# tky823/ssspy

Measured on AMD Instinct MI355X. Metric: GaussILRMA-IP1 update_once mixture-iterations/sec (F=1025,T=512,N=4,K=16), higher is better.
Workload: dtype f64; 1 GPU; BASELINE configs[1] GaussILRMA-IP1/MM (N=M=4, F=1025, T=512, n_basis=16) x 128 independent mixtures per GPU (configs[4] shard), record_loss=False, update_once() = one fused C-ABI call; batch_per_gpu=128, global_batch=128, n_bins=1025, n_frames=512, n_basis=16, parallelism=mixtures sharded, no collective, input=nmf_mixture(seed=1000+b) per mixture b (SURVEY 8d)

## Files before the change

include/ssspy_amd.h:

```cpp
#ifndef SSSPY_AMD_H
#define SSSPY_AMD_H

#include <stddef.h>

#ifdef __cplusplus
extern "C" {
#endif

enum {
  SSSPY_OK = 0,
  SSSPY_ERR_BADARG = 1,
  SSSPY_ERR_HIP = 2,
  SSSPY_ERR_UNSUPPORTED = 3,
  SSSPY_ERR_INTERNAL = 4,
};

enum { SSSPY_FLOOR_NONE = 0, SSSPY_FLOOR_MAX = 1, SSSPY_FLOOR_ADD = 2 };

enum {
  SSSPY_WEIGHT_UNIT = 0,
  SSSPY_WEIGHT_FRAME = 1,
  SSSPY_WEIGHT_BIN_FRAME = 2,
};

// ... 183 lines not shown
int ssspy_ilrma_deferred_logdet_slots(int B, int N, int F, int T, int K, double domain,
                                      int source_model);
int ssspy_ilrma_ip1_update_loss_slots(const void *X, const void *C, void *W, double *basis,
                                      double *activation, void *U, int B, int N, int F, int T,
                                      int K, double domain, int source_model, double model_param,
                                      int normalize, int floor_kind, double floor_eps,
                                      void *workspace, size_t workspace_bytes, int *info,
                                      double *slots, long long slot_stride, double *logdet,
                                      void *stream);
size_t ssspy_fold_scalar_slots_workspace_bytes(long long total, int nslots);
int ssspy_fold_scalar_slots(const double *slots, long long total, int nslots, double *out,
                            void *workspace, size_t workspace_bytes, void *stream);

enum {
  SSSPY_ROUTE_LATENCY = 0,
  SSSPY_ROUTE_THROUGHPUT = 1,
  SSSPY_ROUTE_GROUPED = 2,
  SSSPY_ROUTE_GENERIC = 3,
  SSSPY_ROUTE_WIDE_BASIS = 4,
  SSSPY_ROUTE_RUNTIME_N = 5,
};
int ssspy_ilrma_route(int B, int N, int F, int T, int K, double domain, int source_model,
                      int *act_chunks, int *basis_plan);

int ssspy_ipa_sweep(void *Vc, void *G, int B, int F, int N, int normalization, int max_iter,
                    int floor_kind, double floor_eps, int *info, void *newton_ws,
                    int *not_converged, void *stream);
size_t ssspy_ipa_sweep_newton_words(int B, int N);
int ssspy_debug_barrier_timeouts(void);

int ssspy_ilrma_partition_expand(const double *basis, const double *activation,
                                 const double *latent, double *Teff, double *Vrep, int B, int N,
                                 int F, int T, int K, void *stream);

enum { SSSPY_PARTITION_LATENT = 1, SSSPY_PARTITION_BASIS = 2, SSSPY_PARTITION_ACTIVATION = 4 };

int ssspy_ilrma_partition_update(const void *X, const void *W, double *basis, double *activation,
                                 double *latent, double *Teff, double *Vrep, int B, int N, int F,
                                 int T, int K, double domain, int source_model, double model_param,
                                 int steps, int floor_kind, double floor_eps, void *workspace,
                                 size_t workspace_bytes, void *stream);

int ssspy_ilrma_partition_normalize(void *W, const void *C, void *Y, double *basis, double *latent,
                                    int B, int N, int F, int T, int K, double domain,
                                    int floor_kind, double floor_eps, void *workspace,
                                    size_t workspace_bytes, void *stream);
// ... 450 lines not shown
```

ssspy_amd/_lib.py:

```python

import ctypes
import os

import numpy as np

_PKG = os.path.dirname(os.path.abspath(__file__))
LIB_PATH = os.environ.get("SSSPY_AMD_LIB") or os.path.join(_PKG, "lib", "libssspy_amd.so")

OK, ERR_BADARG, ERR_HIP, ERR_UNSUPPORTED, ERR_INTERNAL = 0, 1, 2, 3, 4
FLOOR_NONE, FLOOR_MAX, FLOOR_ADD = 0, 1, 2
WEIGHT_UNIT, WEIGHT_FRAME, WEIGHT_BIN_FRAME = 0, 1, 2
SOURCE_GAUSS, SOURCE_T, SOURCE_GGD = 0, 1, 2
PARTITION_LATENT, PARTITION_BASIS, PARTITION_ACTIVATION = 1, 2, 4
SOURCE_ME = 0x100
CONTRAST_LAPLACE, CONTRAST_GAUSS, CONTRAST_GAUSS_FIXED = 0, 1, 2
WHITEN, PCA_FIRST_COMPONENT_LAST, PCA_FIRST_COMPONENT_FIRST = 0, 1, 2
IPSDTA_QUAD, IPSDTA_BASIS, IPSDTA_ACT, IPSDTA_COV = range(4)
IPSDTA_MAX_SOURCES, IPSDTA_MAX_BLOCK, IPSDTA_MAX_BASIS = 8, 8, 32
(ROUTE_LATENCY, ROUTE_THROUGHPUT, ROUTE_GROUPED, ROUTE_GENERIC, ROUTE_WIDE_BASIS,
 ROUTE_RUNTIME_N) = range(6)
MNMF_ROUTE_TILED, MNMF_ROUTE_GENERIC, MNMF_ROUTE_RUNTIME = range(3)
MNMF_PLAN_FIELDS = ("fast", "ksmall", "basis_copy", "glds_cov", "glds_spatial", "kq", "handover",
                    "tail_full", "tail_tail", "tail_split", "tail_groups", "htail_full", "htail_tail",
                    "htail_split", "htail_groups", "act_chunks", "ip1_records", "spatial_fold_in_norm",
# ... 70 lines not shown
    "ssspy_ilrma_weighted_covariance": (_i, [_p, _p, _p, _p, _p, _i, _i, _i, _i, _i, _d, _i, _d, _i,
                                             _d, _p, _z, _p]),
    "ssspy_ilrma_normalize_filter": (_i, [_p, _p, _p, _i, _i, _i, _i, _d, _i, _d, _p, _z, _p]),
    "ssspy_ilrma_normalize_output": (_i, [_p, _p, _p, _i, _i, _i, _i, _i, _d, _i, _d, _p, _z, _p]),
    "ssspy_ilrma_normalize_output_tracked": (_i, [_p, _p, _p, _i, _i, _i, _i, _i, _d, _i, _d, _p, _z,
                                                  _p, _p]),
    "ssspy_ilrma_iss_weight": (_i, [_p, _p, _p, _p, _i, _i, _i, _i, _i, _d, _i, _d, _i, _d, _p]),
    "ssspy_ilrma_iss_weight_power": (_i, [_p, _p, _p, _p, _i, _i, _i, _i, _i, _d, _i, _d, _i, _d, _p]),
    "ssspy_ilrma_loss_workspace_bytes": (_z, [_i, _i, _i, _i, _i, _i]),
    "ssspy_ilrma_loss_data": (_i, [_p, _p, _p, _p, _p, _i, _i, _i, _i, _i, _d, _i, _d, _p, _z, _p]),
    "ssspy_ilrma_ip1_update": (_i, [_p, _p, _p, _p, _p, _p, _i, _i, _i, _i, _i, _d, _i, _d, _i, _i, _d,
                                    _p, _z, _p, _p]),
    "ssspy_ilrma_deferred_loss_supported": (_i, [_i, _i, _i, _i, _d, _i]),
    "ssspy_ilrma_ip1_update_deferred_loss": (_i, [_p, _p, _p, _p, _p, _p, _i, _i, _i, _i, _i, _d, _i,
                                                  _d, _i, _i, _d, _p, _z, _p, _p, _p, _p]),
    "ssspy_ilrma_deferred_loss_slots": (_i, [_i, _i, _i, _i, _i, _d, _i]),
    "ssspy_ilrma_deferred_logdet_slots": (_i, [_i, _i, _i, _i, _i, _d, _i]),
    "ssspy_ilrma_ip1_update_loss_slots": (_i, [_p, _p, _p, _p, _p, _p, _i, _i, _i, _i, _i, _d, _i,
                                               _d, _i, _i, _d, _p, _z, _p, _p, _q, _p, _p]),
    "ssspy_fold_scalar_slots_workspace_bytes": (_z, [_q, _i]),
    "ssspy_fold_scalar_slots": (_i, [_p, _q, _i, _p, _p, _z, _p]),
    "ssspy_ilrma_route": (_i, [_i, _i, _i, _i, _i, _d, _i, ctypes.POINTER(ctypes.c_int),
                                ctypes.POINTER(ctypes.c_int)]),
    "ssspy_ilrma_partition_expand": (_i, [_p, _p, _p, _p, _p, _i, _i, _i, _i, _i, _p]),
    "ssspy_ilrma_partition_update": (_i, [_p, _p, _p, _p, _p, _p, _p, _i, _i, _i, _i, _i, _d, _i, _d,
                                          _i, _i, _d, _p, _z, _p]),
    "ssspy_ilrma_partition_normalize": (_i, [_p, _p, _p, _p, _p, _i, _i, _i, _i, _i, _d, _i, _d, _p,
                                             _z, _p]),
    "ssspy_iva_frame_power_workspace_bytes": (_z, [_i, _i, _i, _i]),
    "ssspy_iva_frame_power": (_i, [_p, _p, _p, _i, _i, _i, _i, _p, _z, _p]),
    "ssspy_separate_frame_power": (_i, [_p, _p, _p, _p, _i, _i, _i, _i, _p, _z, _p]),
    "ssspy_iva_weight": (_i, [_p, _p, _p, _i, _i, _i, _i, _i, _i, _d, _p]),
    "ssspy_iva_loss_data": (_i, [_p, _p, _p, _i, _i, _i, _i, _i, _p]),
    "ssspy_iva_score_weight": (_i, [_p, _p, _p, _i, _i, _i, _i, _i, _i, _d, _p]),
    "ssspy_iva_grad_step_logdet_slots": (_i, [_i, _i, _i]),
    "ssspy_iva_grad_step": (_i, [_p, _p, _i, _i, _i, _i, _i, _i, _d, _p, _p, _q, _p]),
    "ssspy_fdica_weight": (_i, [_p, _p, _i, _i, _i, _i, _i, _i, _d, _p, _q, _p]),
    "ssspy_fdica_route": (_i, [_i, _i, _i, _i, _i]),
    "ssspy_fdica_steps": (_i, [_p, _p, _i, _i, _i, _i, _i, _i, _d, _i, _d, _i, _p, _p, _q, _p, _p]),
    "ssspy_ica_chunk_samples": (_i, [_i, _q]),
    "ssspy_ica_workspace_bytes": (_z, [_i, _i, _q]),
    "ssspy_ica_stats": (_i, [_p, _p, _p, _p, _p, _z, _i, _i, _q, _i, _i, _p]),
    "ssspy_ica_step": (_i, [_p, _z, _p, _i, _i, _q, _i, _i, _d, _p, _p, _p, _p, _p]),
    "ssspy_ica_separate": (_i, [_p, _p, _p, _i, _i, _q, _p]),
    "ssspy_prox_neg_logdet": (_i, [_p, _p, _q, _i, _d, _p]),
    "ssspy_pdsbss_contract": (_i, [_p, _p, _p, _i, _i, _i, _i, _i, _p]),
# ... 147 lines not shown
```

ssspy_amd/_ops.py:

```python

from . import _device as dv
from . import _lib, _routes
from ._device import ptr


def _L():
    return _lib.load()


import os as _os

_CANARY_DOUBLES = 4096 if _os.environ.get("SSSPY_AMD_WS_CANARY") else 0
_CANARY_VALUE = -7.25e300
_canaries = []


def _workspace(nbytes, dev):
    n = (int(nbytes) + 7) // 8
    buf = dv.empty((n + _CANARY_DOUBLES,), dv.f64, dev)
    if not _CANARY_DOUBLES:
        return buf, int(nbytes)
    import weakref

    buf[n:].fill_(_CANARY_VALUE)
# ... 491 lines not shown
        ptr(X), ptr(C), ptr(W), ptr(basis), ptr(activation), ptr(U), B, N, F, T, K, domain, model[0],
        model[1], int(bool(normalize)), flooring[0], flooring[1], ptr(ws), ws_bytes, ptr(info),
        ptr(slots), int(slot_stride), ptr(logdet), _st()), "ilrma_ip1_update_loss_slots")


def fold_scalar_slots(slots, total, nslots, out):
    ws, ws_bytes = _scratch(_L().ssspy_fold_scalar_slots_workspace_bytes(int(total), int(nslots)),
                            slots.device)
    _lib.check(_L().ssspy_fold_scalar_slots(ptr(slots), int(total), int(nslots), ptr(out), ptr(ws),
                                            ws_bytes, _st()), "fold_scalar_slots")
    return out


def ilrma_route(B, N, F, T, K, domain, model=GAUSS):
    import ctypes

    chunks = ctypes.c_int(0)
    plan = (ctypes.c_int * 3)()
    route = int(_L().ssspy_ilrma_route(B, N, F, T, K, float(domain), model[0], ctypes.byref(chunks),
                                       plan))
    if route < 0:
        raise ValueError("ilrma_route: bad shape")
    return route, int(chunks.value), tuple(plan)


def ilrma_partition_expand(basis, activation, latent, Teff, Vrep):
    B, N, F, K = Teff.shape
    T = Vrep.shape[-1]
    _lib.check(
        _L().ssspy_ilrma_partition_expand(ptr(basis), ptr(activation), ptr(latent), ptr(Teff),
                                          ptr(Vrep), B, N, F, T, K, _st()),
        "ilrma_partition_expand",
    )


def ilrma_partition_update(X, W, basis, activation, latent, Teff, Vrep, domain, steps, flooring, ws,
                           ws_bytes, model=GAUSS):
    B, N, F, T = X.shape
    K = basis.shape[-1]
    _lib.check(
        _L().ssspy_ilrma_partition_update(ptr(X), ptr(W), ptr(basis), ptr(activation), ptr(latent),
                                          ptr(Teff), ptr(Vrep), B, N, F, T, K, domain, model[0],
                                          model[1], steps, flooring[0], flooring[1], ptr(ws),
                                          ws_bytes, _st()),
        "ilrma_partition_update",
    )
# ... 922 lines not shown
```

ssspy_amd/csrc/ilrma_api.hip:

```cpp
#include "ilrma_plan.hpp"

namespace ssspy {

static inline int check_model(int source_model, double param, double domain = 2.0) {
  const int model = source_model & 0xff;
  const bool me = (source_model & SSSPY_SOURCE_ME) != 0;
  if ((source_model & ~(0xff | SSSPY_SOURCE_ME)) != 0)
    return fail(SSSPY_ERR_BADARG, "bad source model flags");
  if (me && (domain != 2.0 || model == SSSPY_SOURCE_GGD))
    return fail(SSSPY_ERR_BADARG, "ME source updates need domain == 2 and a Gauss or t model");
  if (model == SSSPY_SOURCE_GAUSS) return SSSPY_OK;
  if (model == SSSPY_SOURCE_T && param > 0.0) return SSSPY_OK;
  if (model == SSSPY_SOURCE_GGD && param > 0.0 && param < 2.0) return SSSPY_OK;
  return fail(SSSPY_ERR_BADARG, "bad source model / model_param (t: dof > 0, GGD: 0 < beta < 2)");
}

int ip1_with_power(void *W, const void *U, const void *C, double *qbuf, int B, int F, int N,
                   int floor_kind, double floor_eps, int *info, hipStream_t st);
int separate_power(const void *X, const void *W, double *P, int B, int N, int F, int T,
                   hipStream_t st);
int row_power(const void *W, const void *C, double *qbuf, int B, int F, int N, hipStream_t st);
int wb_update_basis(const double *a, const double *b, double *basis, const double *activation,
                    double *nd, int BN, int F, int T, int K, const IlrmaDims &d, hipStream_t st);
int wb_update_activation(const double *a, const double *b, const double *basis, double *activation,
// ... 772 lines not shown
    int split = 0, rbins = 0;
    auto cov = [&]() -> int {
      ILRMA_FAST_DISPATCH(N, ilrma_fast_wcov, X, W, basis, activation, U, B, F, T, K, ws + w.upart,
                          p.fm_id, p.fm_param, floor_kind, floor_eps, st, &split, &rbins);
    };
    rc = cov();
    if (rc) return rc;
    auto ip1 = [&]() -> int {
      if (loss_data && loss_stride > 0) {
        ILRMA_FAST_DISPATCH(N, ilrma_small_ip1_logdet,
                            split ? (const void *)(ws + w.upart) : (const void *)U, split, rbins, 0ll,
                            normalize ? C : nullptr, W, B, F, floor_kind, floor_eps, qbuf, info,
                            logdet, loss_stride, st);
      }
      ILRMA_FAST_DISPATCH(N, ilrma_small_ip1, split ? (const void *)(ws + w.upart) : (const void *)U,
                          split, rbins, 0ll, normalize ? C : nullptr, W, B, F, floor_kind, floor_eps,
                          qbuf, info, st);
    };
    rc = ip1();
    if (rc || !normalize) return rc;
    ILRMA_FAST_DISPATCH(N, ilrma_small_norm, W, basis, qbuf, B, F, K, domain, floor_kind, floor_eps,
                        st);
  }
  rc = wcov_into(p, w, d, X, W, basis, activation, U, ws, p.power_once ? Xs : nullptr, p.power_once,
                 st);
  if (rc) return rc;
  rc = ip1_with_power(W, U, normalize ? C : nullptr, normalize ? qbuf : nullptr, B, F, N,
                      floor_kind, floor_eps, info, st);
  if (rc || !normalize) return rc;
  return launch_norm_scale(W, basis, qbuf, B, N, F, K, domain, floor_kind, floor_eps, st);
}

int ssspy_ilrma_ip1_update(const void *X, const void *C, void *W, double *basis, double *activation,
                           void *U, int B, int N, int F, int T, int K, double domain,
                           int source_model, double model_param, int normalize, int floor_kind,
                           double floor_eps, void *workspace, size_t workspace_bytes, int *info,
                           void *stream) {
  return ip1_update_impl(X, C, W, basis, activation, U, B, N, F, T, K, domain, source_model,
                         model_param, normalize, floor_kind, floor_eps, workspace, workspace_bytes,
                         info, nullptr, nullptr, stream);
}

int ssspy_ilrma_deferred_loss_supported(int N, int F, int T, int K, double domain,
                                        int source_model) {
  return make_ilrma_plan(1, N, F, T, K, domain, source_model).loss_byproduct;
}

int ssspy_ilrma_ip1_update_deferred_loss(const void *X, const void *C, void *W, double *basis,
                                         double *activation, void *U, int B, int N, int F, int T,
                                         int K, double domain, int source_model, double model_param,
                                         int normalize, int floor_kind, double floor_eps,
// ... 22 lines not shown
                                      void *workspace, size_t workspace_bytes, int *info,
                                      double *slots, long long slot_stride, double *logdet,
                                      void *stream) {
  SSSPY_REQUIRE(slots && logdet && slot_stride >= B && slot_stride < (1ll << 31),
                "ilrma_ip1_update_loss_slots: bad argument");
  return ip1_update_impl(X, C, W, basis, activation, U, B, N, F, T, K, domain, source_model,
                         model_param, normalize, floor_kind, floor_eps, workspace, workspace_bytes,
                         info, slots, logdet, stream, slot_stride);
}

int ssspy_ilrma_route(int B, int N, int F, int T, int K, double domain, int source_model,
                      int *chunks_out, int *basis_plan) {
  if (B <= 0 || N < 2 || N > SSSPY_RT_MAX_SOURCES || F <= 0 || T <= 0 || K < 1 ||
      K > SSSPY_MAX_BASIS || !(domain > 0.0 && domain <= 2.0))
    return -1;
  const IlrmaPlan p = make_ilrma_plan(B, N, F, T, K, domain, source_model);
  if (chunks_out) *chunks_out = p.act_chunks;
  if (basis_plan) {
    basis_plan[0] = p.basis_tail.full;
    basis_plan[1] = p.basis_tail.tail;
    basis_plan[2] = p.basis_tail.split;
  }
  return p.summary;
}

size_t ssspy_fold_scalar_slots_workspace_bytes(long long total, int nslots) {
  if (total <= 0 || nslots <= 0) return 0;
  return align256(fold_scratch_bytes(total, nslots)) + 256;
}

int ssspy_fold_scalar_slots(const double *slots, long long total, int nslots, double *out,
                            void *workspace, size_t workspace_bytes, void *stream) {
  SSSPY_REQUIRE(slots && out && total > 0 && nslots > 0, "fold_scalar_slots: bad argument");
  SSSPY_REQUIRE(workspace && workspace_bytes >= ssspy_fold_scalar_slots_workspace_bytes(total, nslots),
                "fold_scalar_slots: workspace too small");
  return launch_fold_slabs(slots, workspace, out, total, nslots, as_stream(stream), 0);
}

int ssspy_ilrma_partition_expand(const double *basis, const double *activation,
                                 const double *latent, double *Teff, double *Vrep, int B, int N,
                                 int F, int T, int K, void *stream) {
  SSSPY_REQUIRE(basis && activation && latent && Teff && Vrep && B > 0 && N >= 1 && F > 0 &&
                    T > 0 && K >= 1,
                "partition_expand: bad argument");
  const long long per = (long long)K * (F > T ? F : T);
  hipLaunchKernelGGL(k_partition_expand, dim3((unsigned)((per + 255) / 256), N, B), dim3(256), 0,
// ... 106 lines not shown
```

ssspy_amd/csrc/ilrma_fast.hip:

```cpp
#include <cstdlib>

#include "common.hpp"
#include "cov_core.hpp"
#include "fast_model.hpp"
#include "fast_tiles.hpp"
#include "tail_plan.hpp"

#ifndef SSSPY_N
#error "compile with -DSSSPY_N=<n_sources>"
#endif
#if SSSPY_N > 4
#error "fast path is built for n_sources <= 4"
#endif

#define SSSPY_CAT_(a, b) a##b
#define SSSPY_CAT(a, b) SSSPY_CAT_(a, b)
#define LAUNCHER(name) SSSPY_CAT(SSSPY_CAT(name, _n), SSSPY_N)

namespace ssspy {
namespace SSSPY_CAT(ilrma_fast_n, SSSPY_N) {

constexpr int N = SSSPY_N;
using fast::rcp_nr;
using fast::FastModel;
// ... 457 lines not shown

template <int G>
__device__ __forceinline__ void wc_half_store(const double (&acc)[4][WC_HALF], c128 *dst,
                                              double scale) {
  constexpr int PA[2][4][2] = {{{0, 1}, {2, 3}, {0, 0}, {0, 0}}, {{0, 2}, {0, 3}, {1, 2}, {1, 3}}};
  constexpr int NPAIR = G == 0 ? 2 : 4, P0 = G == 0 ? 4 : 0;
#pragma unroll
  for (int n = 0; n < 4; ++n) {
    c128 *d = dst + n * 16;
    if constexpr (G == 0) {
#pragma unroll
      for (int a = 0; a < 4; ++a) d[a * 4 + a] = cmake(acc[n][a] * scale, 0.0);
    }
#pragma unroll
    for (int p = 0; p < NPAIR; ++p) {
      const int a = PA[G][p][0], bb = PA[G][p][1];
      const double zx = acc[n][P0 + 2 * p], zy = acc[n][P0 + 2 * p + 1];
      d[a * 4 + bb] = cmake(zx * scale, zy * scale);
      d[bb * 4 + a] = cmake(zx * scale, -zy * scale);
    }
  }
}

template <int MODEL, int KS, bool FULL = false>
__global__ __launch_bounds__(256, KS >= 16 ? 1 : 2) void k_wcov_fast(const c128 *__restrict__ X,
                                                      const c128 *__restrict__ W,
                                                      const double *__restrict__ basis,
                                                      const double *__restrict__ act,
                                                      c128 *__restrict__ U, int F, int T, int K,
                                                      TailPlan plan, c128 *__restrict__ upart,
                                                      FastModel fm) {
  constexpr int SG = WC_SG;
  constexpr int WSTRIDE = N * N + 1;
  __shared__ __attribute__((aligned(16))) c128 xpatch[4][XPATCH];
  constexpr bool NEEDS_Y = MODEL == FM_T || MODEL == FM_GGD;
  __shared__ __attribute__((aligned(16))) c128 wlc[NEEDS_Y ? 4 * 16 * WSTRIDE : 1];
  constexpr bool SPLIT = WC_SHARE && !NEEDS_Y && MODEL != FM_GAUSSP && KS == 4;
  __shared__ __attribute__((aligned(16))) double phis[SPLIT ? WC_WB * N * 4 * 64 : 1];
  const int lane = threadIdx.x & 63, wave = threadIdx.x >> 6;
  const int c = lane & 15, q = lane >> 4;
  const BlockWork work = block_work(plan);
  const int b = work.b, nchunks = work.nchunks;
  const int g = wave % WC_NG, wb = wave / WC_NG;
  const int s0 = g * SG;
  const int i0 = (work.group * WC_WB + wb) * 16;
  const int bin = min(i0 + c, F - 1);
  const fast::XSrc<N> xsrc = fast::make_xsrc<N>(X + (long long)b * N * F * T, F, T);
  c128 *xshare = &xpatch[0][0] + wb * (N * 16 * 17);
  const double *act_b = act + (long long)b * N * K * T;
  const int ntiles = (T + 15) >> 4;
  const int tpc = (ntiles + nchunks - 1) / nchunks;
  const int jt_begin = work.chunk * tpc, jt_end = min(ntiles, jt_begin + tpc);
  if (wave_idle(i0, F)) {
    if (NEEDS_Y) __syncthreads();
    if constexpr (WC_SHARE) {
      for (int jt = jt_begin; jt < jt_end; ++jt) {
        __syncthreads();
        __syncthreads();
      }
    }
// ... 111 lines not shown
        const double ph = MODEL == FM_GAUSSP ? pow_nonneg(den, -fm.pinv2) : rcp_nr(den);
        phi[s] = (valid && s0 + s < N) ? ph : 0.0;
      }
      if constexpr (!SPLIT) acc.add(x, phi);
    }
  }
  const double scale = 1.0 / (double)T;
  const int ob = i0 + c;
  auto out_bin = [&]() -> c128 * {
    return nchunks == 1 ? U + ((long long)b * F + ob) * (long long)(N * N * N)
                        : upart + (((long long)work.tail_idx * nchunks + work.chunk) * WC_BINS +
                                   (ob - work.group * WC_BINS)) * (long long)(N * N * N);
  };
  if constexpr (SPLIT) {
#pragma unroll
    for (int n = 0; n < 4; ++n)
#pragma unroll
      for (int e = 0; e < WC_HALF; ++e) {
        double v = hacc[n][e];
        v += __shfl_xor(v, 16, 64);
        v += __shfl_xor(v, 32, 64);
        hacc[n][e] = v;
      }
    if (ob < F && q == 0) {
      c128 *dst = out_bin();
      if (gu == 0) wc_half_store<0>(hacc, dst, scale);
      else wc_half_store<1>(hacc, dst, scale);
    }
    return;
  }
  acc.fold_q();
  if (ob < F) {
    c128 *dst = out_bin();
#pragma unroll
    for (int s = 0; s < SG; ++s) {
      const int n = s0 + s;
      if (n < N) {
        int e = 0;
#pragma unroll
        for (int a = 0; a < N; ++a) {
          const bool mine = (a & 3) == q;
          if (mine) dst[(n * N + a) * N + a] = cmake(acc.diag[s][a] * scale, 0.0);
#pragma unroll
          for (int bb = a + 1; bb < N; ++bb) {
            const c128 z = acc.off[s][e];
            if (mine) {
// ... 69 lines not shown
    for (int s = 0; s < SG; ++s) {
      const int n = s0 + s;
      if (n < N) {
        int e = 0;
#pragma unroll
        for (int a = 0; a < N; ++a) {
          const bool mine = (a & 3) == q;
          if (mine) dst[(n * N + a) * N + a] = cmake(acc.diag[s][a] * scale, 0.0);
#pragma unroll
          for (int bb = a + 1; bb < N; ++bb) {
            const c128 z = acc.off[s][e];
            if (mine) {
              dst[(n * N + a) * N + bb] = cmake(z.x * scale, z.y * scale);
              dst[(n * N + bb) * N + a] = cmake(z.x * scale, -z.y * scale);
            }
            ++e;
          }
        }
      }
    }
  }
}

__global__ __launch_bounds__(256) void k_wcov_fold(c128 *__restrict__ U,
                                                   const c128 *__restrict__ upart, int F,
                                                   TailPlan plan) {
  constexpr int PER = WC_BINS * N * N * N;
  const int tail_idx = blockIdx.y;
  const int item = plan.full + tail_idx;
  const int b = item / plan.groups, group = item - b * plan.groups;
  const int e = blockIdx.x * blockDim.x + threadIdx.x;
  const int lb = e / (N * N * N);
  if (e >= PER || group * WC_BINS + lb >= F) return;
  const c128 s2 = ordered_sum(upart + (long long)tail_idx * plan.split * PER + e, (long long)PER,
                              plan.split);
  U[((long long)b * F + group * WC_BINS) * (long long)(N * N * N) + e] = s2;
}

template <int KS>
struct TStage {
  double t[(N * 16 * 4 * KS + 255) / 256];
  c128 w;
};

template <int KS>
constexpr int trow() {
  return 4 * KS + 1;
}

template <int KS, bool FULL>
__device__ __forceinline__ void tstage_load(TStage<KS> &st, const double *__restrict__ basis_b,
                                            const c128 *__restrict__ W_b, int F, int K, int i0) {
  constexpr int KR = 4 * KS;
#pragma unroll
  for (int u = 0; u < (N * 16 * KR + 255) / 256; ++u) {
    const int idx = threadIdx.x + 256 * u;
    const int k = idx % KR, bl = (idx / KR) & 15, n = idx / (16 * KR);
    const int bi = i0 + bl;
    double v = 0.0;
// ... 405 lines not shown
    case FM_GGD: SSSPY_WCOV_LAUNCH(FM_GGD, KS_); break; \
    case FM_GAUSS1: SSSPY_WCOV_LAUNCH(FM_GAUSS1, KS_); break; \
    case FM_GAUSSP: SSSPY_WCOV_LAUNCH(FM_GAUSSP, KS_); break; \
    default: SSSPY_WCOV_LAUNCH(FM_GAUSS, KS_); break;  \
  }
  if (K > 32) {
    SSSPY_WCOV_LAUNCH_M(16)
  } else if (K > 16) {
    SSSPY_WCOV_LAUNCH_M(8)
  } else if (full_tiles(K, T) && fmodel == FM_GAUSS) {
    SSSPY_WCOV_LAUNCH_F(FM_GAUSS, 4, true);
  } else {
    SSSPY_WCOV_LAUNCH_M(4)
  }
#undef SSSPY_WCOV_LAUNCH_M
#undef SSSPY_WCOV_LAUNCH
#undef SSSPY_WCOV_LAUNCH_F
  int rc = check_launch("k_wcov_fast");
  if (rc || plan.tail == 0) return rc;
  if (split_out && plan.full == 0) {
    *split_out = plan.split;
    return rc;
  }
  hipLaunchKernelGGL(k_wcov_fold, dim3((WC_BINS * N * N * N + 255) / 256, plan.tail), block, 0, st,
                     (c128 *)U, (const c128 *)upart, F, plan);
  return check_launch("k_wcov_fold");
}

int LAUNCHER(ilrma_fast_wcov_frame)(const void *X, const double *weight, void *U, int B, int F,
                                    int T, hipStream_t st) {
  static const bool disabled = std::getenv("SSSPY_AMD_NO_FAST") != nullptr;
  const int groups = (F + WC_BINS - 1) / WC_BINS;
  const long long items = (long long)B * groups;
  if (disabled || items < SLOTS || (long long)F * T * 16 >= (1ll << 32)) return -1;
  hipLaunchKernelGGL(k_wcov_frame_fast, dim3((unsigned)items), dim3(256), 0, st, (const c128 *)X,
                     weight, (c128 *)U, F, T, groups);
  return check_launch("k_wcov_frame_fast");
}

#endif

#undef SSSPY_FAST_LAUNCH2
#undef SSSPY_FAST_LAUNCH_M

}
```

ssspy_amd/csrc/ilrma_plan.hpp:

```cpp
#pragma once

#include <cstdlib>

#include "common.hpp"
#include "ilrma_params.hpp"
#include "tail_plan.hpp"
#include "wide_n.hpp"

namespace ssspy {

#define DECL_N(n)                                                                               \
  int ilrma_basis_n##n(const void *, const void *, const double *, double *, const double *,   \
                       IlrmaDims, hipStream_t);                                                \
  int ilrma_activation_n##n(const void *, const void *, const double *, const double *, double *, \
                            int, IlrmaDims, hipStream_t);                                      \
  int ilrma_wcov_n##n(const void *, const void *, const double *, const double *, void *,       \
                      IlrmaDims, hipStream_t);                                                 \
  size_t ilrma_loss_ws_bytes_n##n(int, int);                                                   \
  int ilrma_loss_n##n(const void *, const void *, const double *, const double *, double *,     \
                      void *, IlrmaDims, hipStream_t);
DECL_N(2) DECL_N(3) DECL_N(4) DECL_N(5) DECL_N(6) DECL_N(7) DECL_N(8)
#undef DECL_N

#define DECL_FAST(n)                                                                           \
  int ilrma_fast_basis_n##n(const void *, const void *, const double *, double *, const double *, \
                            int, int, int, int, int, double, double *, int, double, int,        \
                            double *, void *, int, hipStream_t, long long);                     \
  int ilrma_fast_basis_loss_slots_n##n(int, int, int);                                          \
  size_t ilrma_fast_loss_ws_bytes_n##n(int, int);                                               \
  int ilrma_fast_activation_n##n(const void *, const void *, const double *, double *,         \
                                 double *, int, int, int, int, int, int, double, int,           \
                                 hipStream_t, int *, int, int, double);                         \
  int ilrma_fast_wcov_n##n(const void *, const void *, const double *, const double *, void *, \
                           int, int, int, int, void *, int, double, int, double, hipStream_t,  \
                           int *, int *);                                                      \
  int ilrma_fast_loss_n##n(const void *, const void *, const double *, const double *, double *, \
                           void *, int, int, int, int, int, double, hipStream_t);
DECL_FAST(2) DECL_FAST(3) DECL_FAST(4)
#undef DECL_FAST

#define DECL_SMALL(n)                                                                           \
  size_t ilrma_small_scratch_n##n(int, int, int, int);                                            \
  int ilrma_small_activation_n##n(const void *, const void *, const double *, double *, int, int, \
                                  int, int, int, double, double *, int, double, int,              \
                                  hipStream_t);                                                   \
  int ilrma_small_ip1_n##n(const void *, int, int, long long, const void *, void *, int, int, int, \
                           double, double *, int *, hipStream_t);                                 \
  int ilrma_small_ip1_logdet_n##n(const void *, int, int, long long, const void *, void *, int,   \
                                  int, int, double, double *, int *, double *, long long,         \
                                  hipStream_t);                                                   \
  int ilrma_small_norm_n##n(void *, double *, const double *, int, int, int, double, int, double, \
                            hipStream_t);
DECL_SMALL(2) DECL_SMALL(3) DECL_SMALL(4)
#undef DECL_SMALL

bool wide_weighted_cov_ok(int N, int S, int F, int T, int kind);
int wide_weighted_cov(const void *A, const double *weight, int kind, void *U, int B, int N, int S,
                      int F, int T, hipStream_t st);
size_t wb_loss_ws_bytes(int B, int N, int F, int T);

#define ILRMA_FAST_DISPATCH(N_, fn, ...)             \
  switch (N_) {                                      \
// ... 175 lines not shown
  p.cov_tuned = fast;
  p.power_once = p.nmf == NmfRoute::Grouped || p.nmf == NmfRoute::WideBasis;
  p.ip1_latency = small;
  p.weights_buf = N > 4 || wide;
  p.dense_buf = wide;
  p.summary = p.runtime_n                      ? SSSPY_ROUTE_RUNTIME_N
              : p.nmf == NmfRoute::Grouped     ? SSSPY_ROUTE_GROUPED
              : small                          ? SSSPY_ROUTE_LATENCY
              : p.nmf == NmfRoute::WideBasis   ? SSSPY_ROUTE_WIDE_BASIS
              : tuned                          ? SSSPY_ROUTE_THROUGHPUT
                                               : SSSPY_ROUTE_GENERIC;
  return p;
}

static inline CovRoute cov_route(const IlrmaPlan &p, bool ysep, bool filter) {
  const bool weights_ok = p.gauss || ysep || !filter;
  if (p.runtime_n) return CovRoute::RuntimeN;
  if (p.K > 32 && weights_ok) return CovRoute::WideBasis;
  if (p.cov_matrix_core && weights_ok) return CovRoute::MatrixCore;
  if (p.cov_tuned && (p.gauss || filter)) return CovRoute::Tuned;
  return CovRoute::Generic;
}

static inline IlrmaPlan shape_plan(int B, int N, int F, int T, int K) {
  return make_ilrma_plan(B, N, F, T, K, 2.0, SSSPY_SOURCE_GAUSS);
}

static inline size_t loss_slots_bytes(const IlrmaPlan &p, int B, int F, int T, bool with_filter) {
  const int N = p.N;
  const size_t a = generic_loss_ws_bytes(B, N, F), b = tuned_loss_ws_bytes(B, N, F);
  size_t c = p.runtime_n ? rt_ilrma_loss_ws_bytes(B, N, F) : 0;
  if (p.loss == LossRoute::WideBasis) {
    const size_t g = align256(wb_loss_ws_bytes(B, N, F, T)) +
                     (with_filter ? align256((size_t)B * N * F * T * sizeof(double)) : 0);
    c = c > g ? c : g;
  }
  return align256(a > b ? (a > c ? a : c) : (b > c ? b : c));
}

struct IlrmaWs {
  size_t act_part, btmp, qbuf, psi, lslots, bpart, upart, praw, ybuf, wbuf, gb, gnd, total;
};
static inline size_t qbuf_bytes(int B, int N, int F) {
  return align256((size_t)B * F * N * sizeof(double));
}
static inline IlrmaWs ilrma_ws(int B, int N, int F, int T, int K) {
// ... 36 lines not shown
```

ssspy_amd/csrc/spatial_kernels.hip:

```cpp
#include <cstdlib>

#include "common.hpp"
#include "cov_core.hpp"
#include "smallmat.hpp"
#include "wide_n.hpp"

namespace ssspy {
int ilrma_fast_wcov_frame_n2(const void *, const double *, void *, int, int, int, hipStream_t);
int ilrma_fast_wcov_frame_n3(const void *, const double *, void *, int, int, int, hipStream_t);
int ilrma_fast_wcov_frame_n4(const void *, const double *, void *, int, int, int, hipStream_t);

bool wide_weighted_cov_ok(int N, int S, int F, int T, int kind);
int wide_weighted_cov(const void *A, const double *weight, int kind, void *U, int B, int N, int S,
                      int F, int T, hipStream_t st);

thread_local char g_last_error[512] = "";

template <int N, bool POWER = false>
__global__ __launch_bounds__(256) void k_separate(const c128 *__restrict__ X,
                                                  const c128 *__restrict__ W, c128 *Y, int F,
                                                  int T) {
  const int i = blockIdx.x, b = blockIdx.y;
  const c128 *__restrict__ w = W + ((long long)b * F + i) * (N * N);
  const long long row0 = ((long long)b * N) * F + i;
// ... 278 lines not shown
    qf = qf < 0.0 ? 0.0 : qf;
    const double d = apply_floor(sqrt(qf), floor_kind, eps);
#pragma unroll
    for (int r = 0; r < N; ++r)
#pragma unroll
      for (int c = 0; c < N; ++c)
        if (r == n) Wm.a[r][c] = cmake(w[c].x / d, -w[c].y / d);
  }
  store_mat<N>(Wm, W + idx * (N * N));
  if (!ok && info) atomicAdd(info, 1);
  if (C && qbuf) {
    Mat<N> Cm;
    load_mat<N>(Cm, C + idx * (N * N));
#pragma unroll
    for (int n = 0; n < N; ++n) {
      c128 v[N];
#pragma unroll
      for (int m = 0; m < N; ++m) v[m] = cconj(Wm.a[n][m]);
      qbuf[idx * N + n] = quad_form<N>(v, Cm);
    }
  }
}

template <int N>
__global__ __launch_bounds__(64) void k_ip1_source_solve(c128 *W, const c128 *__restrict__ U,
                                                         double *__restrict__ denom,
                                                         long long nbins, int n, int *info) {
  const long long idx = (long long)blockIdx.x * blockDim.x + threadIdx.x;
  if (idx >= nbins) return;
  Mat<N> Wm, Un, A;
  load_mat<N>(Wm, W + idx * (N * N));
  load_mat<N>(Un, U + (idx * N + n) * (N * N));
  matmul<N>(A, Wm, Un);
  c128 w[N];
  const bool ok = solve_unit<N>(A, n, w);
  double qf = quad_form<N>(w, Un);
  qf = qf < 0.0 ? 0.0 : qf;
  denom[idx] = sqrt(qf);
#pragma unroll
  for (int c = 0; c < N; ++c) W[idx * (N * N) + n * N + c] = cconj(w[c]);
  if (!ok && info) atomicAdd(info, 1);
}

__global__ __launch_bounds__(256) void k_scale_filter_row(c128 *W, const double *__restrict__ denom,
                                                          long long nbins, int N, int n) {
  const long long e = (long long)blockIdx.x * blockDim.x + threadIdx.x;
// ... 339 lines not shown
}

int ip1_with_power(void *W, const void *U, const void *C, double *qbuf, int B, int F, int N,
                   int floor_kind, double floor_eps, int *info, hipStream_t st) {
  const long long nbins = (long long)B * F;
  if (rt_sources_ok(N)) return rt_ip1(W, U, C, qbuf, B, F, N, floor_kind, floor_eps, info, st);
  if (ip1_small_shape(B, F, N))
    return ip1_from_records(W, U, 0, 0, 0, C, qbuf, B, F, N, floor_kind, floor_eps, info, st, nullptr, 0);
  dim3 grid((unsigned)((nbins + 63) / 64)), block(64);
  if (N > 4) {
    dim3 g8((unsigned)((nbins * 8 + 255) / 256)), b8(256);
    switch (N) {
      case 5: hipLaunchKernelGGL((k_ip1_rows<5, 8>), g8, b8, 0, st, (c128 *)W, (const c128 *)U, nbins, floor_kind, floor_eps, info, (const c128 *)C, qbuf); break;
      case 6: hipLaunchKernelGGL((k_ip1_rows<6, 8>), g8, b8, 0, st, (c128 *)W, (const c128 *)U, nbins, floor_kind, floor_eps, info, (const c128 *)C, qbuf); break;
      case 7: hipLaunchKernelGGL((k_ip1_rows<7, 8>), g8, b8, 0, st, (c128 *)W, (const c128 *)U, nbins, floor_kind, floor_eps, info, (const c128 *)C, qbuf); break;
      case 8: hipLaunchKernelGGL((k_ip1_rows<8, 8>), g8, b8, 0, st, (c128 *)W, (const c128 *)U, nbins, floor_kind, floor_eps, info, (const c128 *)C, qbuf); break;
      default: return fail(SSSPY_ERR_UNSUPPORTED, "n_sources must be in [1, 8]");
    }
    return check_launch("k_ip1_rows");
  }
  DISPATCH_N4(N, hipLaunchKernelGGL((k_ip1<NN>), grid, block, 0, st, (c128 *)W, (const c128 *)U,
                                    nbins, floor_kind, floor_eps, info, (const c128 *)C, qbuf));
  return check_launch("k_ip1");
}

int separate_power(const void *X, const void *W, double *P, int B, int N, int F, int T,
                   hipStream_t st) {
  if (rt_sources_ok(N)) return rt_separate(X, W, P, B, N, F, T, true, st);
  dim3 grid(F, B), block(256);
  DISPATCH_N(N, hipLaunchKernelGGL((k_separate<NN, true>), grid, block, 0, st, (const c128 *)X,
                                   (const c128 *)W, (c128 *)P, F, T));
  return check_launch("k_separate_power");
}

int row_power(const void *W, const void *C, double *qbuf, int B, int F, int N, hipStream_t st) {
  if (rt_sources_ok(N)) return rt_row_power(W, C, qbuf, B, F, N, st);
  const long long nbins = (long long)B * F;
  dim3 grid((unsigned)((nbins + 63) / 64)), block(64);
  DISPATCH_N(N, hipLaunchKernelGGL((k_row_power<NN>), grid, block, 0, st, (const c128 *)W,
                                   (const c128 *)C, qbuf, nbins));
  return check_launch("k_row_power");
}
}

extern "C" {

// ... 254 lines not shown
```

ssspy_amd/csrc/tail_plan.hpp:

```cpp
#pragma once

#include "common.hpp"

namespace ssspy {

constexpr int SLOTS = 512;
struct TailPlan {
  int full, tail, split, groups;
};

static inline int best_split(long long items, int ntiles, int slots, int max_split,
                             long long max_blocks) {
  if (items <= 0 || ntiles <= 1) return 1;
  const double ovh = 2.0, fold = 0.15;
  int best = 1;
  double best_cost = (double)((items + slots - 1) / slots) * (ntiles + ovh);
  if (max_split > ntiles) max_split = ntiles;
  for (int s = 2; s <= max_split; ++s) {
    const int tpc = (ntiles + s - 1) / s;
    const int se = (ntiles + tpc - 1) / tpc;
    if (se != s) continue;
    const long long blocks = items * se;
    if (blocks > max_blocks) break;
    const double cost = (double)((blocks + slots - 1) / slots) * (tpc + ovh) + fold * se;
// ... 11 lines not shown
  const long long items = (long long)B * groups;
  p.groups = groups;
  p.full = (int)(items / slots) * slots;
  p.tail = (int)(items - p.full);
  p.split = p.tail > 0 ? best_split(p.tail, ntiles, slots, 16, max_blocks > 0 ? max_blocks : slots) : 1;
  if (p.split == 1) {
    p.full += p.tail;
    p.tail = 0;
  }
  return p;
}

static inline TailPlan ilrma_basis_plan(int B, int F, int T, int K) {
  const int ktiles = K > 32 ? 4 : (K > 16 ? 2 : 1);
#ifdef SSSPY_KTILE_ITEMS
  const int item_tiles = ktiles;
#else
  const int item_tiles = ktiles == 2 ? 1 : ktiles;
#endif
  return make_tail_plan(B, ((F + 63) / 64) * item_tiles, (T + 15) / 16, ktiles >= 2 ? 256 : SLOTS,
                        ktiles >= 2 ? 256 : 1024);
}

struct BlockWork {
  int b, group, chunk, nchunks, tail_idx;
};
__device__ __forceinline__ BlockWork block_work(const TailPlan &p) {
  BlockWork w;
  int item = blockIdx.x;
  if (item < p.full) item = xcd_contiguous(item, p.full);
  w.chunk = 0;
  w.nchunks = 1;
  w.tail_idx = 0;
  if (item >= p.full) {
    const int t = item - p.full;
    w.tail_idx = t / p.split;
    w.chunk = t - w.tail_idx * p.split;
    w.nchunks = p.split;
    item = p.full + w.tail_idx;
  }
  w.b = item / p.groups;
  w.group = item - w.b * p.groups;
  return w;
}

}
// ... 1 lines not shown
```

Baseline: 42300 iterations/s.

## Store IP1 weighted covariances as packed Hermitian records for N=4

New measurement: 42620 iterations/s, median of 6. No clear change (+0.7%).

```diff
diff --git a/include/ssspy_amd.h b/include/ssspy_amd.h
--- a/include/ssspy_amd.h
+++ b/include/ssspy_amd.h
@@ -229,6 +229,9 @@
 };
 int ssspy_ilrma_route(int B, int N, int F, int T, int K, double domain, int source_model,
                       int *act_chunks, int *basis_plan);
+
+int ssspy_ilrma_ip1_record(int B, int N, int F, int T, int K, double domain, int source_model,
+                           int *cov_plan);
 
 int ssspy_ipa_sweep(void *Vc, void *G, int B, int F, int N, int normalization, int max_iter,
                     int floor_kind, double floor_eps, int *info, void *newton_ws,
diff --git a/ssspy_amd/_lib.py b/ssspy_amd/_lib.py
--- a/ssspy_amd/_lib.py
+++ b/ssspy_amd/_lib.py
@@ -116,6 +116,7 @@
     "ssspy_fold_scalar_slots": (_i, [_p, _q, _i, _p, _p, _z, _p]),
     "ssspy_ilrma_route": (_i, [_i, _i, _i, _i, _i, _d, _i, ctypes.POINTER(ctypes.c_int),
                                 ctypes.POINTER(ctypes.c_int)]),
+    "ssspy_ilrma_ip1_record": (_i, [_i, _i, _i, _i, _i, _d, _i, ctypes.POINTER(ctypes.c_int)]),
     "ssspy_ilrma_partition_expand": (_i, [_p, _p, _p, _p, _p, _i, _i, _i, _i, _i, _p]),
     "ssspy_ilrma_partition_update": (_i, [_p, _p, _p, _p, _p, _p, _p, _i, _i, _i, _i, _i, _d, _i, _d,
                                           _i, _i, _d, _p, _z, _p]),
diff --git a/ssspy_amd/_ops.py b/ssspy_amd/_ops.py
--- a/ssspy_amd/_ops.py
+++ b/ssspy_amd/_ops.py
@@ -537,6 +537,16 @@
     if route < 0:
         raise ValueError("ilrma_route: bad shape")
     return route, int(chunks.value), tuple(plan)
+
+
+def ilrma_ip1_record(B, N, F, T, K, domain, model=GAUSS):
+    import ctypes
+
+    plan = (ctypes.c_int * 3)()
+    packed = int(_L().ssspy_ilrma_ip1_record(B, N, F, T, K, float(domain), model[0], plan))
+    if packed < 0:
+        raise ValueError("ilrma_ip1_record: bad shape")
+    return bool(packed), tuple(plan)
 
 
 def ilrma_partition_expand(basis, activation, latent, Teff, Vrep):
diff --git a/ssspy_amd/csrc/ilrma_api.hip b/ssspy_amd/csrc/ilrma_api.hip
--- a/ssspy_amd/csrc/ilrma_api.hip
+++ b/ssspy_amd/csrc/ilrma_api.hip
@@ -818,11 +818,18 @@
     ILRMA_FAST_DISPATCH(N, ilrma_small_norm, W, basis, qbuf, B, F, K, domain, floor_kind, floor_eps,
                         st);
   }
-  rc = wcov_into(p, w, d, X, W, basis, activation, U, ws, p.power_once ? Xs : nullptr, p.power_once,
-                 st);
-  if (rc) return rc;
-  rc = ip1_with_power(W, U, normalize ? C : nullptr, normalize ? qbuf : nullptr, B, F, N,
-                      floor_kind, floor_eps, info, st);
+  if (packed_record(p, B, F)) {
+    rc = ilrma_fast_wcov_packed_n4(X, basis, activation, U, B, F, T, K, ws + w.upart, p.fm_id, st);
+    if (rc) return rc;
+    rc = ip1_packed_with_power(W, U, normalize ? C : nullptr, normalize ? qbuf : nullptr, B, F,
+                               floor_kind, floor_eps, info, st);
+  } else {
+    rc = wcov_into(p, w, d, X, W, basis, activation, U, ws, p.power_once ? Xs : nullptr,
+                   p.power_once, st);
+    if (rc) return rc;
+    rc = ip1_with_power(W, U, normalize ? C : nullptr, normalize ? qbuf : nullptr, B, F, N,
+                        floor_kind, floor_eps, info, st);
+  }
   if (rc || !normalize) return rc;
   return launch_norm_scale(W, basis, qbuf, B, N, F, K, domain, floor_kind, floor_eps, st);
 }
@@ -891,6 +898,21 @@
     basis_plan[2] = p.basis_tail.split;
   }
   return p.summary;
+}
+
+int ssspy_ilrma_ip1_record(int B, int N, int F, int T, int K, double domain, int source_model,
+                           int *cov_plan) {
+  if (B <= 0 || N < 2 || N > SSSPY_RT_MAX_SOURCES || F <= 0 || T <= 0 || K < 1 ||
+      K > SSSPY_MAX_BASIS || !(domain > 0.0 && domain <= 2.0))
+    return -1;
+  const bool packed = packed_record(make_ilrma_plan(B, N, F, T, K, domain, source_model), B, F);
+  if (cov_plan) {
+    const TailPlan t = packed ? packed_cov_plan(B, F, T) : TailPlan{0, 0, 1, 0};
+    cov_plan[0] = t.full;
+    cov_plan[1] = t.tail;
+    cov_plan[2] = t.split;
+  }
+  return packed ? 1 : 0;
 }
 
 size_t ssspy_fold_scalar_slots_workspace_bytes(long long total, int nslots) {
diff --git a/ssspy_amd/csrc/ilrma_fast.hip b/ssspy_amd/csrc/ilrma_fast.hip
--- a/ssspy_amd/csrc/ilrma_fast.hip
+++ b/ssspy_amd/csrc/ilrma_fast.hip
@@ -503,7 +503,19 @@
   }
 }
 
-template <int MODEL, int KS, bool FULL = false>
+constexpr int WC_REC = 16;
+template <int G>
+__device__ __forceinline__ void wc_half_store_packed(const double (&acc)[4][WC_HALF], double *dst,
+                                                     double scale) {
+#pragma unroll
+  for (int n = 0; n < 4; ++n) {
+    c128 *d = (c128 *)(dst + n * WC_REC + G * WC_HALF);
+#pragma unroll
+    for (int e = 0; e < WC_HALF; e += 2) d[e >> 1] = cmake(acc[n][e] * scale, acc[n][e + 1] * scale);
+  }
+}
+
+template <int MODEL, int KS, bool FULL = false, bool PACKED = false>
 __global__ __launch_bounds__(256, KS >= 16 ? 1 : 2) void k_wcov_fast(const c128 *__restrict__ X,
                                                       const c128 *__restrict__ W,
                                                       const double *__restrict__ basis,
@@ -517,6 +529,7 @@
   constexpr bool NEEDS_Y = MODEL == FM_T || MODEL == FM_GGD;
   __shared__ __attribute__((aligned(16))) c128 wlc[NEEDS_Y ? 4 * 16 * WSTRIDE : 1];
   constexpr bool SPLIT = WC_SHARE && !NEEDS_Y && MODEL != FM_GAUSSP && KS == 4;
+  static_assert(SPLIT || !PACKED, "the packed record is the split form's");
   __shared__ __attribute__((aligned(16))) double phis[SPLIT ? WC_WB * N * 4 * 64 : 1];
   const int lane = threadIdx.x & 63, wave = threadIdx.x >> 6;
   const int c = lane & 15, q = lane >> 4;
@@ -674,6 +687,18 @@
         v += __shfl_xor(v, 32, 64);
         hacc[n][e] = v;
       }
+    if constexpr (PACKED) {
+      if (ob < F && q == 0) {
+        double *dst = nchunks == 1
+                          ? (double *)U + ((long long)b * F + ob) * (long long)(N * WC_REC)
+                          : (double *)upart +
+                                (((long long)work.tail_idx * nchunks + work.chunk) * WC_BINS +
+                                 (ob - work.group * WC_BINS)) * (long long)(N * WC_REC);
+        if (gu == 0) wc_half_store_packed<0>(hacc, dst, scale);
+        else wc_half_store_packed<1>(hacc, dst, scale);
+      }
+      return;
+    }
     if (ob < F && q == 0) {
       c128 *dst = out_bin();
       if (gu == 0) wc_half_store<0>(hacc, dst, scale);
@@ -789,19 +814,20 @@
   }
 }
 
+template <int PB = N * N * N>
 __global__ __launch_bounds__(256) void k_wcov_fold(c128 *__restrict__ U,
                                                    const c128 *__restrict__ upart, int F,
                                                    TailPlan plan) {
-  constexpr int PER = WC_BINS * N * N * N;
+  constexpr int PER = WC_BINS * PB;
   const int tail_idx = blockIdx.y;
   const int item = plan.full + tail_idx;
   const int b = item / plan.groups, group = item - b * plan.groups;
   const int e = blockIdx.x * blockDim.x + threadIdx.x;
-  const int lb = e / (N * N * N);
+  const int lb = e / PB;
   if (e >= PER || group * WC_BINS + lb >= F) return;
   const c128 s2 = ordered_sum(upart + (long long)tail_idx * plan.split * PER + e, (long long)PER,
                               plan.split);
-  U[((long long)b * F + group * WC_BINS) * (long long)(N * N * N) + e] = s2;
+  U[((long long)b * F + group * WC_BINS) * (long long)PB + e] = s2;
 }
 
 template <int KS>
@@ -1253,10 +1279,41 @@
     *split_out = plan.split;
     return rc;
   }
-  hipLaunchKernelGGL(k_wcov_fold, dim3((WC_BINS * N * N * N + 255) / 256, plan.tail), block, 0, st,
+  hipLaunchKernelGGL(k_wcov_fold<>, dim3((WC_BINS * N * N * N + 255) / 256, plan.tail), block, 0, st,
                      (c128 *)U, (const c128 *)upart, F, plan);
   return check_launch("k_wcov_fold");
 }
+
+#if SSSPY_N == 4
+int ilrma_fast_wcov_packed_n4(const void *X, const double *basis, const double *act, void *rec,
+                              int B, int F, int T, int K, void *upart, int fmodel,
+                              hipStream_t st) {
+  if (K > 16 || !(fmodel == FM_GAUSS || fmodel == FM_GAUSS1))
+    return fail(SSSPY_ERR_INTERNAL, "wcov_packed: shape off the component split");
+  static_assert(WC_BINS == PACKED_BINS, "packed_cov_plan() is this pass's plan");
+  const TailPlan plan = packed_cov_plan(B, F, T);
+  const FastModel fm = make_fast_model(fmodel, 0.0, 0, SSSPY_FLOOR_NONE, 0.0);
+  dim3 grid(plan.full + plan.tail * plan.split), block(256);
+#define SSSPY_WCOV_LAUNCH_P(M, FULL_)                                                             \
+  hipLaunchKernelGGL((k_wcov_fast<M, 4, FULL_, true>), grid, block, 0, st, (const c128 *)X,        \
+                     (const c128 *)nullptr, basis, act, (c128 *)rec, F, T, K, plan, (c128 *)upart, \
+                     fm)
+  if (fmodel == FM_GAUSS1) {
+    SSSPY_WCOV_LAUNCH_P(FM_GAUSS1, false);
+  } else if (full_tiles(K, T)) {
+    SSSPY_WCOV_LAUNCH_P(FM_GAUSS, true);
+  } else {
+    SSSPY_WCOV_LAUNCH_P(FM_GAUSS, false);
+  }
+#undef SSSPY_WCOV_LAUNCH_P
+  int rc = check_launch("k_wcov_fast");
+  if (rc || plan.tail == 0) return rc;
+  constexpr int PB = N * WC_REC / 2;
+  hipLaunchKernelGGL(k_wcov_fold<PB>, dim3((WC_BINS * PB + 255) / 256, plan.tail), block, 0, st,
+                     (c128 *)rec, (const c128 *)upart, F, plan);
+  return check_launch("k_wcov_fold");
+}
+#endif
 
 int LAUNCHER(ilrma_fast_wcov_frame)(const void *X, const double *weight, void *U, int B, int F,
                                     int T, hipStream_t st) {
diff --git a/ssspy_amd/csrc/ilrma_plan.hpp b/ssspy_amd/csrc/ilrma_plan.hpp
--- a/ssspy_amd/csrc/ilrma_plan.hpp
+++ b/ssspy_amd/csrc/ilrma_plan.hpp
@@ -38,6 +38,10 @@
                            void *, int, int, int, int, int, double, hipStream_t);
 DECL_FAST(2) DECL_FAST(3) DECL_FAST(4)
 #undef DECL_FAST
+int ilrma_fast_wcov_packed_n4(const void *, const double *, const double *, void *, int, int, int,
+                              int, void *, int, hipStream_t);
+int ip1_packed_with_power(void *W, const void *rec, const void *C, double *qbuf, int B, int F,
+                          int floor_kind, double floor_eps, int *info, hipStream_t st);
 
 #define DECL_SMALL(n)                                                                           \
   size_t ilrma_small_scratch_n##n(int, int, int, int);                                            \
@@ -259,6 +263,13 @@
   return CovRoute::Generic;
 }
 
+bool ip1_small_shape(int B, int F, int N);
+static inline bool packed_record(const IlrmaPlan &p, int B, int F) {
+  return p.N == 4 && p.K <= 16 && (p.fm_id == 0 || p.fm_id == 3) && p.nmf == NmfRoute::Tuned &&
+         !p.ip1_latency && cov_route(p, false, true) == CovRoute::Tuned &&
+         !ip1_small_shape(B, F, p.N);
+}
+
 static inline IlrmaPlan shape_plan(int B, int N, int F, int T, int K) {
   return make_ilrma_plan(B, N, F, T, K, 2.0, SSSPY_SOURCE_GAUSS);
 }
diff --git a/ssspy_amd/csrc/spatial_kernels.hip b/ssspy_amd/csrc/spatial_kernels.hip
--- a/ssspy_amd/csrc/spatial_kernels.hip
+++ b/ssspy_amd/csrc/spatial_kernels.hip
@@ -324,6 +324,66 @@
   }
 }
 
+__device__ __forceinline__ void unpack_herm4(Mat<4> &m, const c128 (&r)[8]) {
+  const double d[4] = {r[0].x, r[0].y, r[1].x, r[1].y};
+  constexpr int PA[6][2] = {{0, 1}, {2, 3}, {0, 2}, {0, 3}, {1, 2}, {1, 3}};
+#pragma unroll
+  for (int a = 0; a < 4; ++a) m.a[a][a] = cmake(d[a], 0.0);
+#pragma unroll
+  for (int p = 0; p < 6; ++p) {
+    m.a[PA[p][0]][PA[p][1]] = r[2 + p];
+    m.a[PA[p][1]][PA[p][0]] = cmake(r[2 + p].x, -r[2 + p].y);
+  }
+}
+
+__global__ __launch_bounds__(64) void k_ip1_packed(c128 *W, const c128 *__restrict__ rec,
+                                                   long long nbins, int floor_kind, double eps,
+                                                   int *info, const c128 *__restrict__ C,
+                                                   double *qbuf) {
+  constexpr int N = 4;
+  const long long idx = (long long)blockIdx.x * blockDim.x + threadIdx.x;
+  if (idx >= nbins) return;
+  const c128 *mine = rec + idx * (N * 8);
+  c128 nxt[8];
+#pragma unroll
+  for (int e = 0; e < 8; ++e) nxt[e] = mine[e];
+  Mat<N> Wm;
+  load_mat<N>(Wm, W + idx * (N * N));
+  bool ok = true;
+#pragma unroll 1
+  for (int n = 0; n < N; ++n) {
+    Mat<N> Un, A;
+    unpack_herm4(Un, nxt);
+    const int n1 = n + 1 < N ? n + 1 : n;
+#pragma unroll
+    for (int e = 0; e < 8; ++e) nxt[e] = mine[n1 * 8 + e];
+    matmul<N>(A, Wm, Un);
+    c128 w[N];
+    ok = solve_unit<N>(A, n, w) && ok;
+    double qf = quad_form<N>(w, Un);
+    qf = qf < 0.0 ? 0.0 : qf;
+    const double d = apply_floor(sqrt(qf), floor_kind, eps);
+#pragma unroll
+    for (int r = 0; r < N; ++r)
+#pragma unroll
+      for (int c = 0; c < N; ++c)
+        if (r == n) Wm.a[r][c] = cmake(w[c].x / d, -w[c].y / d);
+  }
+  store_mat<N>(Wm, W + idx * (N * N));
+  if (!ok && info) atomicAdd(info, 1);
+  if (C && qbuf) {
+    Mat<N> Cm;
+    load_mat<N>(Cm, C + idx * (N * N));
+#pragma unroll
+    for (int n = 0; n < N; ++n) {
+      c128 v[N];
+#pragma unroll
+      for (int m = 0; m < N; ++m) v[m] = cconj(Wm.a[n][m]);
+      qbuf[idx * N + n] = quad_form<N>(v, Cm);
+    }
+  }
+}
+
 template <int N>
 __global__ __launch_bounds__(64) void k_ip1_source_solve(c128 *W, const c128 *__restrict__ U,
                                                          double *__restrict__ denom,
@@ -709,6 +769,14 @@
   DISPATCH_N4(N, hipLaunchKernelGGL((k_ip1<NN>), grid, block, 0, st, (c128 *)W, (const c128 *)U,
                                     nbins, floor_kind, floor_eps, info, (const c128 *)C, qbuf));
   return check_launch("k_ip1");
+}
+
+int ip1_packed_with_power(void *W, const void *rec, const void *C, double *qbuf, int B, int F,
+                          int floor_kind, double floor_eps, int *info, hipStream_t st) {
+  const long long nbins = (long long)B * F;
+  hipLaunchKernelGGL(k_ip1_packed, dim3((unsigned)((nbins + 63) / 64)), dim3(64), 0, st, (c128 *)W,
+                     (const c128 *)rec, nbins, floor_kind, floor_eps, info, (const c128 *)C, qbuf);
+  return check_launch("k_ip1_packed");
 }
 
 int separate_power(const void *X, const void *W, double *P, int B, int N, int F, int T,
diff --git a/ssspy_amd/csrc/tail_plan.hpp b/ssspy_amd/csrc/tail_plan.hpp
--- a/ssspy_amd/csrc/tail_plan.hpp
+++ b/ssspy_amd/csrc/tail_plan.hpp
@@ -57,6 +57,11 @@
                         ktiles >= 2 ? 256 : 1024);
 }
 
+constexpr int PACKED_BINS = 32;
+static inline TailPlan packed_cov_plan(int B, int F, int T) {
+  return make_tail_plan(B, (F + PACKED_BINS - 1) / PACKED_BINS, (T + 15) / 16, SLOTS, 1024);
+}
+
 struct BlockWork {
   int b, group, chunk, nchunks, tail_idx;
 };
```
